# jasperlinthorst/reveal

Hardware: AMD Instinct MI355X
Metric: Mbp/s indexed+MUM-anchored (reveal rem) (higher is better)
Workload: dtype int32

## Files before the change

### reveal_amd/csrc/rv_cascade.hip

```cpp
#include "rv_index.h"
#include "rv_cascade.h"
#include "rv_leaf.h"
#include <algorithm>
#include <string.h>
#include <stdio.h>
#include <stdlib.h>
#include <chrono>

namespace {

constexpr int TB = 256;
constexpr u32 NONE = 0xFFFFFFFFu;
#ifdef RV_SA64
constexpr int KEY_SHIFT = 40;
#else
constexpr int KEY_SHIFT = 32;
#endif
constexpr u64 KEY_LOW = (1ull << KEY_SHIFT) - 1;

struct CasIv { sa_t a0, a1, b0, b1; };
struct CasRes { sa_t qa, qb; u32 ql, lead, trail, state; };
enum { C_NCHILD = 0, C_NUND = 1, C_NWIT = 2, C_ERR = 3, C_MAXN = 4, C_LO = 5, C_HI = 6, C_LEVELS = 7, C_NSOLVED = 8, C_NUNSOLVED = 9, C_NRETRY = 10, C_TICKET = 11,
       C_NANCH = 12  };

__device__ inline bool cas_cut(const CasIv &iv, int64_t pa, int64_t pb, int64_t len, int64_t minl, int64_t *qa, int64_t *qb, int64_t *ql) {
    const int64_t ka = (int64_t)iv.a0 - pa, kb = (int64_t)iv.b0 - pb;
    int64_t k = ka > kb ? ka : kb;
    k = k > 0 ? k : 0;
    const int64_t a = pa + k, b = pb + k;
    int64_t l = len - k;
    const int64_t ra = (int64_t)iv.a1 - a, rb = (int64_t)iv.b1 - b;
    l = l < ra ? l : ra;
    l = l < rb ? l : rb;
    *qa = a; *qb = b; *ql = l;
    return l >= minl;
}
__device__ inline u64 cas_key(int64_t qa, int64_t ql) { return ((u64)ql << KEY_SHIFT) | (KEY_LOW - (u64)qa); }

__device__ inline u64 shfl_up64(u64 v, int d) {
    const u32 lo = __shfl_up((u32)v, d, 64), hi = __shfl_up((u32)(v >> 32), d, 64);
    return ((u64)hi << 32) | lo;
}
__device__ inline void seg_atomic_max64(u64 *__restrict__ dst, u32 child, u64 val, bool active) {
    const int lane = threadIdx.x & 63;
    if (!active) { child = NONE; val = 0; }
    val = rv_wave_seg_max_u64(child, val);
    const u32 nc = __shfl_down(child, 1, 64);
    const bool last = lane == 63 || nc != child;
    if (active && last && val > dst[child]) atomicMax((unsigned long long *)&dst[child], (unsigned long long)val);
}
__device__ inline void seg_atomic_max32(u32 *__restrict__ dst, u32 child, u32 val, bool active) {
    const int lane = threadIdx.x & 63;
    if (!active) { child = NONE; val = 0; }
    val = rv_wave_seg_max_u32(child, val);
    const u32 nc = __shfl_down(child, 1, 64);
    const bool last = lane == 63 || nc != child;
    if (active && last && val > dst[child]) atomicMax(&dst[child], val);
}

constexpr int WT_ITEMS = 8;
constexpr int WT_TILE = TB * WT_ITEMS;
constexpr int WT_REGIONS = RV_WIT_REGIONS;
__global__ __launch_bounds__(TB) void k_cas_witness(const sa_t *__restrict__ SA, const lcp_t *__restrict__ LCP, const uint8_t *__restrict__ BWT, int64_t n,
                                                    u32 minl, sa_t *__restrict__ w_pos, u32 *__restrict__ w_val, u32 *__restrict__ w_rank, u32 cap , u32 *__restrict__ counters ) {
    __shared__ __attribute__((aligned(16))) u32 sl0[WT_TILE + 8];
    __shared__ __attribute__((aligned(16))) uint8_t ss0[WT_TILE + 32];
    u32 *const sl = sl0 + 3;
    uint8_t *const ss = ss0 + 15;
    const int64_t j0 = (int64_t)blockIdx.x * WT_TILE;
    if (j0 + WT_TILE + 2 <= n && sizeof(lcp_t) == 4) {
        const uint4 *L4 = reinterpret_cast<const uint4 *>(LCP + j0);
        uint4 *d4 = reinterpret_cast<uint4 *>(sl + 1);
        for (int k = threadIdx.x; k < WT_TILE / 4; k += TB) d4[k] = L4[k];
        const uint4 *B4 = reinterpret_cast<const uint4 *>(BWT + j0);
        for (int k = threadIdx.x; k < WT_TILE / 16; k += TB) {
            uint4 v = B4[k];
            v.x = (v.x >> 7) & 0x01010101u; v.y = (v.y >> 7) & 0x01010101u; v.z = (v.z >> 7) & 0x01010101u; v.w = (v.w >> 7) & 0x01010101u;
            reinterpret_cast<uint4 *>(ss + 1)[k] = v;
        }
        if (threadIdx.x == 0) { sl[0] = j0 > 0 ? (u32)LCP[j0 - 1] : 0u; ss[0] = j0 > 0 ? (uint8_t)(BWT[j0 - 1] >> 7) : (uint8_t)0; }
        if (threadIdx.x == 1) { sl[WT_TILE + 1] = (u32)LCP[j0 + WT_TILE]; ss[WT_TILE + 1] = (uint8_t)(BWT[j0 + WT_TILE] >> 7); }
        if (threadIdx.x == 2) sl[WT_TILE + 2] = (u32)LCP[j0 + WT_TILE + 1];
    } else {
        for (int k = threadIdx.x; k < WT_TILE + 3; k += TB) { const int64_t j = j0 - 1 + k; sl[k] = (j >= 0 && j < n) ? (u32)LCP[j] : 0u; }
        for (int k = threadIdx.x; k < WT_TILE + 2; k += TB) { const int64_t j = j0 - 1 + k; ss[k] = (j >= 0 && j < n) ? (uint8_t)(BWT[j] >> 7) : (uint8_t)0; }
    }
    __syncthreads();
    const int lane = threadIdx.x & 63;
    const u64 lt = (lane == 0) ? 0ull : (~0ull >> (64 - lane));
#pragma unroll 1
// ... 101 lines not shown
    if (i < NW) {
        const int64_t pos = (int64_t)w_pos[i];
        const bool a_side = t.nB == 0 || pos < (int64_t)t.beginB[0];
        const int ct = a_side ? cas_contig_of(t.beginA, t.nA, pos) : cas_contig_of(t.beginB, t.nB, pos);
        u32 c = NONE;
        if (ct >= 0) {
            const int32_t k = a_side ? t.pickA[ct] : t.pickB[ct];
            if (k >= 0) {
                for (int which = 0; which < 2 && c == NONE; which++) {
                    const u32 r = which ? t.rootTrail[k] : t.rootLead[k];
                    if (r == NONE) continue;
                    const CasIv p = roots[r];
                    if ((pos >= (int64_t)p.a0 && pos < (int64_t)p.a1) || (pos >= (int64_t)p.b0 && pos < (int64_t)p.b1)) c = r;
                }
            }
        }
        w_child[i] = c;
    }
}
__global__ void k_cas_lineage_stats(unsigned long long *__restrict__ stats, unsigned long long steps, unsigned long long maxdepth) {
    if (threadIdx.x == 0 && blockIdx.x == 0) { atomicAdd(&stats[0], steps); atomicMax(&stats[3], maxdepth); }
}
__global__ __launch_bounds__(TB) void k_cas_lkeys(const sa_t *__restrict__ c_pa, const u32 *__restrict__ c_len, u32 M, u64 *__restrict__ keys, u32 *__restrict__ vals) {
    const u32 i = blockIdx.x * TB + threadIdx.x;
    if (i < M) { keys[i] = (((1ull << (64 - KEY_SHIFT)) - 1ull - (u64)c_len[i]) << KEY_SHIFT) | (u64)c_pa[i]; vals[i] = i; }
}
__global__ __launch_bounds__(TB) void k_cas_lgather(const sa_t *__restrict__ c_pa, const sa_t *__restrict__ c_pb, const u32 *__restrict__ c_len, const u32 *__restrict__ perm, u32 M,
                                                    sa_t *__restrict__ o_pa, sa_t *__restrict__ o_pb, u32 *__restrict__ o_len) {
    const u32 i = blockIdx.x * TB + threadIdx.x;
    if (i < M) { const u32 f = perm[i]; o_pa[i] = c_pa[f]; o_pb[i] = c_pb[f]; o_len[i] = c_len[f]; }
}

constexpr int CAS_ITEMS = 4;
__global__ __launch_bounds__(TB) void k_cas_assign(const sa_t *__restrict__ c_pa, const sa_t *__restrict__ c_pb, const u32 *__restrict__ c_len, u32 *__restrict__ c_child,
                                                   u32 M, const sa_t *__restrict__ w_pos, const u32 *__restrict__ w_val, u32 *__restrict__ w_child, u32 NW,
                                                   const CasIv *__restrict__ iv, const CasRes *__restrict__ res, u64 *__restrict__ best, u32 *__restrict__ wmax,
                                                   int64_t minl, int first, const u64 *__restrict__ ceil ) {
    const u32 mblocks = (M + TB * CAS_ITEMS - 1) / (TB * CAS_ITEMS);
    for (int it = 0; it < CAS_ITEMS; it++) {
    if (blockIdx.x < mblocks) {
        const u32 i = (blockIdx.x * CAS_ITEMS + (u32)it) * TB + threadIdx.x;
        u32 c = i < M ? c_child[i] : NONE;
        bool live = c != NONE;
        u64 key = 0;
        if (live) {
            const int64_t pa = (int64_t)c_pa[i], pb = (int64_t)c_pb[i], len = (int64_t)c_len[i];
            int64_t qa, qb, ql;
            if (!first) {
                const CasRes r = res[c];
                const CasIv p = iv[c];
                u32 nc = NONE;
                if (r.state == 1u) {
                    CasIv lv; lv.a0 = p.a0; lv.a1 = r.qa; lv.b0 = p.b0; lv.b1 = r.qb;
                    CasIv tv; tv.a0 = (sa_t)((int64_t)r.qa + r.ql); tv.a1 = p.a1; tv.b0 = (sa_t)((int64_t)r.qb + r.ql); tv.b1 = p.b1;
                    if (r.lead != NONE && cas_cut(lv, pa, pb, len, minl, &qa, &qb, &ql)) nc = r.lead;
                    else if (r.trail != NONE && cas_cut(tv, pa, pb, len, minl, &qa, &qb, &ql)) nc = r.trail;
                } else if (r.state == 3u) {
                    if (cas_cut(p, pa, pb, len, minl, &qa, &qb, &ql)) nc = r.lead;
                }
                c = nc;
                c_child[i] = c;
                live = c != NONE;
            } else {
                live = cas_cut(iv[c], pa, pb, len, minl, &qa, &qb, &ql);
                if (!live) { c = NONE; c_child[i] = NONE; }
            }
            if (live) key = cas_key(qa, ql);
        }
        bool bid = live;
        if (live && ceil) { const u64 ce = ceil[c]; bid = ce == 0 || key < ce; }
        seg_atomic_max64(best, c, key, bid);
    } else {
        const u32 i = ((blockIdx.x - mblocks) * CAS_ITEMS + (u32)it) * TB + threadIdx.x;
        u32 c = i < NW ? w_child[i] : NONE;
        bool live = c != NONE;
        u32 v = 0;
        if (live) {
            const int64_t pos = (int64_t)w_pos[i];
            v = w_val[i];
            if (!first) {
                const CasRes r = res[c];
                const CasIv p = iv[c];
                u32 nc = NONE;
                if (r.state == 1u) {
                    const int64_t ea = (int64_t)r.qa + r.ql, eb = (int64_t)r.qb + r.ql;
                    const bool in_lead = (pos >= p.a0 && pos < r.qa) || (pos >= p.b0 && pos < r.qb);
                    const bool in_trail = (pos >= ea && pos < p.a1) || (pos >= eb && pos < p.b1);
                    nc = in_lead ? r.lead : in_trail ? r.trail : NONE;
                } else if (r.state == 3u) nc = r.lead;
                c = nc;
                w_child[i] = c;
                live = c != NONE;
            } else {
                const CasIv p = iv[c];
                live = (pos >= p.a0 && pos < p.a1) || (pos >= p.b0 && pos < p.b1);
                if (!live) { c = NONE; w_child[i] = NONE; }
            }
        }
        seg_atomic_max32(wmax, c, v, live);
    }
    }
}

__global__ __launch_bounds__(TB) void k_cas_winner(const sa_t *__restrict__ c_pa, const sa_t *__restrict__ c_pb, const u32 *__restrict__ c_len,
                                                   const u32 *__restrict__ c_child, u32 M, const CasIv *__restrict__ iv, CasRes *__restrict__ res,
                                                   const u64 *__restrict__ best, int64_t minl) {
    const u32 i = blockIdx.x * TB + threadIdx.x;
    if (i >= M) return;
    const u32 c = c_child[i];
    if (c == NONE) return;
    int64_t qa, qb, ql;
    if (!cas_cut(iv[c], (int64_t)c_pa[i], (int64_t)c_pb[i], (int64_t)c_len[i], minl, &qa, &qb, &ql)) return;
    if (cas_key(qa, ql) == best[c]) { res[c].qa = (sa_t)qa; res[c].qb = (sa_t)qb; res[c].ql = (u32)ql; }
}

constexpr u32 DWALK = 1024;
struct CasDanger { u64 *best; u32 *flag; sa_t *qb; u64 *ceil; u32 *m1, *p1, *m2; u64 *key; const uint8_t *T0; const lcp_t *LCP; const u64 *rank; u32 leaf_n; uint8_t *dflag; const uint8_t *wcls; };
__device__ inline bool cas_is_danger(const CasIv &p, u64 bk, u32 wm, u32 minl, u32 leaf_n, u32 *theta) {
    const int64_t la = (int64_t)p.a1 - p.a0, lb = (int64_t)p.b1 - p.b0;
    const u32 bl = (u32)(bk >> KEY_SHIFT);
    const bool can = (la >= (int64_t)minl) & (lb >= (int64_t)minl);
    const bool split = can & (bl >= minl) & (bl > wm);
    *theta = bl >= minl ? bl : minl;
    return can & !split & (wm >= minl) & ((u64)(la + lb) > (u64)leaf_n);
}
__global__ __launch_bounds__(TB) void k_cas_dmark(const CasIv *__restrict__ iv, const u64 *__restrict__ best, const u32 *__restrict__ wmax, u32 minl, const u32 *__restrict__ counters, CasDanger dg) {
    const u32 lo = counters[C_LO], hi = counters[C_HI];
    for (u32 id = lo + blockIdx.x * TB + threadIdx.x; id < hi; id += gridDim.x * TB) {
        u32 theta;
        dg.dflag[id] = cas_is_danger(iv[id], best[id], wmax[id], minl, dg.leaf_n, &theta) ? 1 : 0;
    }
}
__global__ __launch_bounds__(TB) void k_cas_dwalk(const sa_t *__restrict__ w_pos, const u32 *__restrict__ w_val, const u32 *__restrict__ w_child, u32 NW,
                                                  const CasIv *__restrict__ iv, const u64 *__restrict__ best, const u32 *__restrict__ wmax, u32 minl, CasDanger dg) {
    const u32 i = blockIdx.x * TB + threadIdx.x;
    if (i >= NW) return;
    if (dg.wcls && dg.wcls[i]) return;
    const u32 c = w_child[i];
    if (c == NONE || !dg.dflag[c]) return;
    dg.m1[i] = 0; dg.key[i] = 0;
    const CasIv p = iv[c];
    u32 theta;
    if (!cas_is_danger(p, best[c], wmax[c], minl, dg.leaf_n, &theta)) return;
    const int64_t pos = (int64_t)w_pos[i];
    const int64_t cap = (pos < (int64_t)p.a1 ? (int64_t)p.a1 : (int64_t)p.b1) - pos;
    if (w_val[i] < theta || cap < (int64_t)theta) return;
    u32 b1 = 0, b2 = 0, part = NONE;
    bool over = false;
#pragma unroll 1
    for (int dir = -1; dir <= 1; dir += 2) {
        u32 steps = 0;
        u64 rk = dg.rank[i];
        u32 run = 0xFFFFFFFFu;
        for (int64_t k = (int64_t)i + dir; k >= 0 && k < (int64_t)NW; k += dir) {
            const u64 r2 = dg.rank[k];
            if (r2 != rk + (u64)(int64_t)dir) break;
            const u32 g = (u32)dg.LCP[dir > 0 ? r2 : rk];
            run = g < run ? g : run;
            rk = r2;
            if (run < theta) break;
            if (++steps > DWALK) { over = true; break; }
            if (w_child[k] != c || w_val[k] < theta) continue;
            const int64_t pk = (int64_t)w_pos[k];
            const int64_t ck = (pk < (int64_t)p.a1 ? (int64_t)p.a1 : (int64_t)p.b1) - pk;
            if (ck < (int64_t)theta) continue;
            u32 l = (u32)(cap < ck ? cap : ck);
            l = run < l ? run : l;
            if (l > b1) { b2 = b1; b1 = l; part = (u32)k; }
            else if (l > b2) b2 = l;
// ... 3 lines not shown
    if (over) atomicOr(&dg.flag[c], 2u);
    dg.m1[i] = b1 >= theta ? b1 : 0u; dg.p1[i] = part; dg.m2[i] = b2;
}
constexpr u32 BLK_MIN = 64, BLK_MAX = 1024;
__global__ __launch_bounds__(TB) void k_cas_blk_flags(const u64 *__restrict__ rank, const lcp_t *__restrict__ LCP, u32 NW, u32 minl, u32 *__restrict__ flag) {
    const u32 i = blockIdx.x * TB + threadIdx.x;
    if (i >= NW) return;
    flag[i] = (i == 0 || rank[i] != rank[i - 1] + 1 || (u32)LCP[rank[i]] < minl) ? 1u : 0u;
}
__global__ __launch_bounds__(TB) void k_cas_blk_off(const u32 *__restrict__ flag, const u32 *__restrict__ bid, u32 NW, u32 nb, u32 *__restrict__ boff) {
    const u32 i = blockIdx.x * TB + threadIdx.x;
    if (i == 0) boff[nb] = NW;
    if (i < NW && flag[i]) boff[bid[i]] = i;
}
__global__ __launch_bounds__(TB) void k_cas_blk_class(const u32 *__restrict__ flag, const u32 *__restrict__ bid, const u32 *__restrict__ boff, u32 NW, u32 *__restrict__ mflag, uint8_t *__restrict__ wcls) {
    const u32 i = blockIdx.x * TB + threadIdx.x;
    if (i >= NW) return;
    const u32 b = bid[i] + flag[i] - 1u;
    const u32 size = boff[b + 1] - boff[b];
    const bool med = size > BLK_MIN && size <= BLK_MAX;
    wcls[i] = med ? 1 : 0;
    if (flag[i]) mflag[b] = med ? 1u : 0u;
}
__global__ __launch_bounds__(TB) void k_cas_blk_list(const u32 *__restrict__ mflag, const u32 *__restrict__ mid, u32 nb, u32 *__restrict__ mlist) {
    const u32 b = blockIdx.x * TB + threadIdx.x;
    if (b < nb && mflag[b]) mlist[mid[b]] = b;
}
__global__ __launch_bounds__(TB) void k_cas_dwalk_blk(const sa_t *__restrict__ w_pos, const u32 *__restrict__ w_val, const u32 *__restrict__ w_child, const u32 *__restrict__ boff,
                                                      const u32 *__restrict__ mlist, u32 nmed, const CasIv *__restrict__ iv, const u64 *__restrict__ best, const u32 *__restrict__ wmax,
                                                      u32 minl, CasDanger dg) {
    __shared__ u32 cc[BLK_MAX], vv[BLK_MAX], ll[BLK_MAX];
    __shared__ sa_t pp[BLK_MAX];
    __shared__ u32 s_any;
    const u32 b = mlist[blockIdx.x];
    const u32 s0 = boff[b], size = boff[b + 1] - s0;
    if (threadIdx.x == 0) s_any = 0;
    __syncthreads();
    bool any = false;
    for (u32 j = threadIdx.x; j < size; j += TB) {
        const u32 c = w_child[s0 + j];
        cc[j] = c;
        any |= c != NONE && dg.dflag[c];
    }
    if (__ballot(any) && (threadIdx.x & 63) == 0) s_any = 1;
    __syncthreads();
    if (!s_any) return;
    for (u32 j = threadIdx.x; j < size; j += TB) {
        vv[j] = w_val[s0 + j]; pp[j] = w_pos[s0 + j];
        ll[j] = (u32)dg.LCP[dg.rank[s0 + j]];
    }
    __syncthreads();
    for (u32 j = threadIdx.x; j < size; j += TB) {
        const u32 c = cc[j];
        if (c == NONE || !dg.dflag[c]) continue;
        const u32 i = s0 + j;
        dg.m1[i] = 0; dg.key[i] = 0;
        const CasIv p = iv[c];
        u32 theta;
        if (!cas_is_danger(p, best[c], wmax[c], minl, dg.leaf_n, &theta)) continue;
        const int64_t pos = (int64_t)pp[j];
        const int64_t cap = (pos < (int64_t)p.a1 ? (int64_t)p.a1 : (int64_t)p.b1) - pos;
        if (vv[j] < theta || cap < (int64_t)theta) continue;
        u32 b1 = 0, b2 = 0, part = NONE;
#pragma unroll 1
        for (int dir = -1; dir <= 1; dir += 2) {
            u32 run = 0xFFFFFFFFu;
            for (int64_t k = (int64_t)j + dir; k >= 0 && k < (int64_t)size; k += dir) {
                const u32 g = ll[dir > 0 ? k : k + 1];
                run = g < run ? g : run;
                if (run < theta) break;
                if (cc[k] != c || vv[k] < theta) continue;
                const int64_t pk = (int64_t)pp[k];
                const int64_t ck = (pk < (int64_t)p.a1 ? (int64_t)p.a1 : (int64_t)p.b1) - pk;
                if (ck < (int64_t)theta) continue;
                u32 l = (u32)(cap < ck ? cap : ck);
                l = run < l ? run : l;
                if (l > b1) { b2 = b1; b1 = l; part = s0 + (u32)k; }
                else if (l > b2) b2 = l;
                if (run <= b2) break;
            }
        }
        dg.m1[i] = b1 >= theta ? b1 : 0u; dg.p1[i] = part; dg.m2[i] = b2;
    }
}
__global__ __launch_bounds__(TB) void k_cas_dpick(const sa_t *__restrict__ w_pos, const u32 *__restrict__ w_val, const u32 *__restrict__ w_child, u32 NW,
                                                  const CasIv *__restrict__ iv, const CasRes *__restrict__ res, const u64 *__restrict__ best, const u32 *__restrict__ wmax,
                                                  u32 minl, CasDanger dg) {
    const u32 i = blockIdx.x * TB + threadIdx.x;
    if (i >= NW) return;
    const u32 c = w_child[i];
    if (c == NONE || !dg.dflag[c]) return;
    const CasIv p = iv[c];
    u32 theta;
    const u64 bk = best[c];
    if (!cas_is_danger(p, bk, wmax[c], minl, dg.leaf_n, &theta)) return;
    const int64_t pos = (int64_t)w_pos[i];
    const int64_t cap = (pos < (int64_t)p.a1 ? (int64_t)p.a1 : (int64_t)p.b1) - pos;
    if (w_val[i] < theta || cap < (int64_t)theta) return;
    if ((u32)(bk >> KEY_SHIFT) >= minl) { const CasRes r = res[c]; if (pos == (int64_t)r.qa || pos == (int64_t)r.qb) atomicOr(&dg.flag[c], 1u); }
    const u32 b1 = dg.m1[i];
    if (b1 == 0) return;
    const u32 w = dg.p1[i];
    if (dg.m1[w] != b1 || dg.p1[w] != i || b1 <= dg.m2[i] || b1 <= dg.m2[w]) return;
    const int64_t pw = (int64_t)w_pos[w];
    const bool a_side = pos < (int64_t)p.a1, w_a_side = pw < (int64_t)p.a1;
    if (!a_side || w_a_side) return;
    const int64_t qa = pos, qb = pw;
    if (!(qa == (int64_t)p.a0 || qb == (int64_t)p.b0)) {
        const uint8_t ca = dg.T0[qa - 1];
        if (ca == dg.T0[qb - 1] && ca != 'N' && ca != '$' && !(ca >= 'a' && ca <= 'z')) return;
    }
    const u64 key = cas_key(qa, (int64_t)b1);
    dg.key[i] = key;
    if (key > dg.best[c]) atomicMax((unsigned long long *)&dg.best[c], (unsigned long long)key);
}
__global__ __launch_bounds__(TB) void k_cas_dwrite(const sa_t *__restrict__ w_pos, const u32 *__restrict__ w_child, u32 NW, CasDanger dg) {
    const u32 i = blockIdx.x * TB + threadIdx.x;
    if (i >= NW) return;
    const u32 c = w_child[i];
    if (c == NONE || !dg.dflag[c]) return;
    const u64 key = dg.key[i];
    if (key == 0) return;
    if (key == dg.best[c]) dg.qb[c] = w_pos[dg.p1[i]];
}

__global__ __launch_bounds__(TB) void k_cas_decide(CasIv *__restrict__ iv, u64 *__restrict__ best, u32 *__restrict__ wmax, int32_t *__restrict__ depth,
                                                   CasRes *__restrict__ res, u32 minl, u32 *__restrict__ counters, u32 child_cap,
                                                   u32 *__restrict__ und_list, u32 leaf_n, RvCascadeIO io, CasDanger dg, int danger) {
    __shared__ u32 s_cnt[TB / 64][3];
    __shared__ u32 s_base[3];
    const u32 lo = counters[C_LO], hi = counters[C_HI];
    const int lane = threadIdx.x & 63, w = threadIdx.x >> 6;
    const u64 lt = (lane == 0) ? 0ull : (~0ull >> (64 - lane));
    for (u32 first = lo + blockIdx.x * TB; first < hi; first += gridDim.x * TB) {
        const u32 id = first + threadIdx.x;
        const bool in = id < hi;
        CasIv p; p.a0 = p.a1 = p.b0 = p.b1 = 0;
        u64 bk = 0; u32 wm = 0; int32_t dp = 0;
        CasRes r; r.qa = r.qb = 0; r.ql = 0; r.lead = r.trail = NONE; r.state = 2;
        if (in) { p = iv[id]; bk = best[id]; wm = wmax[id]; dp = depth[id]; r = res[id]; }
        const int64_t la = (int64_t)p.a1 - p.a0, lb = (int64_t)p.b1 - p.b0;
        const u32 bl = (u32)(bk >> KEY_SHIFT);
        const bool can = in & (la >= (int64_t)minl) & (lb >= (int64_t)minl);
        bool split = can & (bl >= minl) & (bl > wm);
        bool und = can & !split & (wm >= minl);
        bool forced = false, retry = false;
        if (danger && und && (u64)(la + lb) > (u64)dg.leaf_n) {
            const u32 fl = dg.flag[id];
            const u64 kh = dg.best[id], kc = (bl >= minl && !(fl & 1u)) ? bk : 0ull;
            if (!(fl & 2u)) {
                if (kh == 0 && kc == 0) {
                    if (bl < minl) und = false;
                    else if ((fl >> 8) < 16u) { retry = true; und = false; }
                } else {
                    if (kh > kc) { r.qa = (sa_t)(KEY_LOW - (kh & KEY_LOW)); r.qb = dg.qb[id]; r.ql = (u32)(kh >> KEY_SHIFT); }
                    split = true; forced = true; und = false;
                }
            }
// ... 512 lines not shown
            }
        }
        dg.leaf_n = (u32)ws.opt.cascade_danger_min;
    }
    const sa_t *d_beginA = nullptr, *d_beginB = nullptr;
    if (!chain) {
        hipLaunchKernelGGL(k_cas_init, dim3((unsigned)std::max<int64_t>(1, ceil_div((int64_t)NW, TB))), dim3(TB), 0, q, biv.as<CasIv>(), bbest.as<u64>(), bwm.as<u32>(),
                           bdep.as<int32_t>(), bres.as<CasRes>(), counters, root, bwc.as<u32>(), NW, dg.best, dg.flag, dg.ceil);
        RV_LAUNCH_CHECK();
    } else {
        const u32 R = cb.lin_roots, P = cb.lin_picks;
        if ((int64_t)R + 16 > (int64_t)ccap_k || P > iok.anchor_cap) GIVE_UP("more sequences than the cascade's tables hold");
        const uint8_t *tb = cb.d[32].as<uint8_t>();
        CasRootTabs rt;
        rt.beginA = (const sa_t *)(tb + cb.lin_off[0]); rt.beginB = (const sa_t *)(tb + cb.lin_off[1]);
        rt.pickA = (const int32_t *)(tb + cb.lin_off[2]); rt.pickB = (const int32_t *)(tb + cb.lin_off[3]);
        rt.rootLead = (const u32 *)(tb + cb.lin_off[4]); rt.rootTrail = (const u32 *)(tb + cb.lin_off[5]);
        rt.nA = cb.lin_nA; rt.nB = cb.lin_nB;
        d_beginA = rt.beginA; d_beginB = rt.beginB;
        hipLaunchKernelGGL(k_cas_init_roots, dim3((unsigned)std::max<int64_t>(1, ceil_div((int64_t)R, TB))), dim3(TB), 0, q, biv.as<CasIv>(), bbest.as<u64>(), bwm.as<u32>(),
                           bdep.as<int32_t>(), bres.as<CasRes>(), counters, (const CasIv *)cb.d[30].as<CasIv>(), (const int32_t *)cb.d[31].as<int32_t>(), R, dg.best, dg.flag, dg.ceil);
        RV_LAUNCH_CHECK();
        hipLaunchKernelGGL(k_cas_assign_roots, dim3((unsigned)std::max<int64_t>(1, ceil_div((int64_t)std::max(M, NW), TB))), dim3(TB), 0, q, (const sa_t *)bpa.as<sa_t>(),
                           (const sa_t *)bpb.as<sa_t>(), (const u32 *)blen.as<u32>(), bcc.as<u32>(), M, wp, bwc.as<u32>(), NW, (const CasIv *)cb.d[30].as<CasIv>(), rt, (int64_t)minl);
        RV_LAUNCH_CHECK();
        RV_HIP(hipMemcpyAsync(io.anchor_pos, cb.d[33].p, (size_t)P * 16, hipMemcpyDeviceToDevice, q));
        RV_HIP(hipMemcpyAsync(io.anchor_l, (const uint8_t *)cb.d[33].p + (size_t)P * 16, (size_t)P * 4, hipMemcpyDeviceToDevice, q));
        RV_HIP(hipMemcpyAsync(io.anchor_count, &cb.lin_picks, 4, hipMemcpyHostToDevice, q));
    }

    if (verbose) { (void)hipStreamSynchronize(q); tp[2] = cas_now(); }
    const unsigned agrid = (unsigned)(ceil_div((int64_t)M, TB * CAS_ITEMS) + ceil_div((int64_t)NW, TB * CAS_ITEMS));
    const int batch = std::max(1, (int)ws.opt.cascade_batch);
    int queued = 0;
    RV_TRY(rv_working_text_begin(h, host ? host->side : nullptr));
    u32 sent = 0, known = 0;
    auto send_known = [&]() -> int {
        if (!host || !host->side || !host->l || known <= sent || known > host->cap) return 0;
        RV_HIP(hipMemcpyAsync(host->pos + 2 * (size_t)sent, io.anchor_pos + 2 * (size_t)sent, (size_t)(known - sent) * 16, hipMemcpyDeviceToHost, host->side));
        RV_HIP(hipMemcpyAsync(host->l + sent, io.anchor_l + sent, (size_t)(known - sent) * 4, hipMemcpyDeviceToHost, host->side));
        sent = known;
        return 0;
    };
    struct PrioScope {
        Workspace &w; hipStream_t home; RvCascadeBufs &cb; bool on = false;
        ~PrioScope() { leave(); }
        void leave() {
            if (!on) return;
            on = false;
            (void)hipEventRecord(cb.ev_out, w.stream);
            w.stream = home;
            (void)hipStreamWaitEvent(home, cb.ev_out, 0);
        }
    } prio{ws, q, cb};
    if (ws.opt.cascade_prio) {
        if (!cb.prio_stream) {
            int plo = 0, phi = 0;
            RV_HIP(hipDeviceGetStreamPriorityRange(&plo, &phi));
            RV_HIP(hipStreamCreateWithPriority(&cb.prio_stream, hipStreamNonBlocking, phi));
            RV_HIP(hipEventCreateWithFlags(&cb.ev_in, hipEventDisableTiming));
            RV_HIP(hipEventCreateWithFlags(&cb.ev_out, hipEventDisableTiming));
        }
        RV_HIP(hipEventRecord(cb.ev_in, q));
        RV_HIP(hipStreamWaitEvent(cb.prio_stream, cb.ev_in, 0));
        ws.stream = cb.prio_stream; prio.on = true;
        q = cb.prio_stream;
    }
    for (;;) {
        for (int b = 0; b < batch; b++, queued++) {
            hipLaunchKernelGGL(k_cas_assign, dim3(agrid), dim3(TB), 0, q, (const sa_t *)bpa.as<sa_t>(), (const sa_t *)bpb.as<sa_t>(), (const u32 *)blen.as<u32>(), bcc.as<u32>(), M,
                               wp, wv, bwc.as<u32>(), NW, (const CasIv *)biv.as<CasIv>(), (const CasRes *)bres.as<CasRes>(),
                               bbest.as<u64>(), bwm.as<u32>(), (int64_t)minl, queued == 0 ? 1 : 0, (const u64 *)((danger && NW) ? dg.ceil : nullptr));
            RV_LAUNCH_CHECK();
            hipLaunchKernelGGL(k_cas_winner, dim3((unsigned)ceil_div((int64_t)M, TB)), dim3(TB), 0, q, (const sa_t *)bpa.as<sa_t>(), (const sa_t *)bpb.as<sa_t>(),
                               (const u32 *)blen.as<u32>(), (const u32 *)bcc.as<u32>(), M, (const CasIv *)biv.as<CasIv>(), bres.as<CasRes>(), (const u64 *)bbest.as<u64>(), (int64_t)minl);
            RV_LAUNCH_CHECK();
            if (danger && NW) {
                const unsigned wb = (unsigned)ceil_div((int64_t)NW, TB);
                hipLaunchKernelGGL(k_cas_dmark, dim3(256), dim3(TB), 0, q, (const CasIv *)biv.as<CasIv>(), (const u64 *)bbest.as<u64>(), (const u32 *)bwm.as<u32>(), minl, (const u32 *)counters, dg);
                RV_LAUNCH_CHECK();
                hipLaunchKernelGGL(k_cas_dwalk, dim3(wb), dim3(TB), 0, q, wp, wv, (const u32 *)bwc.as<u32>(), NW, (const CasIv *)biv.as<CasIv>(), (const u64 *)bbest.as<u64>(),
                                   (const u32 *)bwm.as<u32>(), minl, dg);
                RV_LAUNCH_CHECK();
                if (dwalk_nmed) {
                    hipLaunchKernelGGL(k_cas_dwalk_blk, dim3((unsigned)dwalk_nmed), dim3(TB), 0, q, wp, wv, (const u32 *)bwc.as<u32>(), dwalk_boff, dwalk_mlist, dwalk_nmed,
                                       (const CasIv *)biv.as<CasIv>(), (const u64 *)bbest.as<u64>(), (const u32 *)bwm.as<u32>(), minl, dg);
                    RV_LAUNCH_CHECK();
                }
                hipLaunchKernelGGL(k_cas_dpick, dim3(wb), dim3(TB), 0, q, wp, wv, (const u32 *)bwc.as<u32>(), NW, (const CasIv *)biv.as<CasIv>(), (const CasRes *)bres.as<CasRes>(),
                                   (const u64 *)bbest.as<u64>(), (const u32 *)bwm.as<u32>(), minl, dg);
                RV_LAUNCH_CHECK();
                hipLaunchKernelGGL(k_cas_dwrite, dim3(wb), dim3(TB), 0, q, wp, (const u32 *)bwc.as<u32>(), NW, dg);
                RV_LAUNCH_CHECK();
            }
            hipLaunchKernelGGL(k_cas_decide, dim3(256), dim3(TB), 0, q, biv.as<CasIv>(), bbest.as<u64>(), bwm.as<u32>(), bdep.as<int32_t>(),
                               bres.as<CasRes>(), minl, counters, ccap_k, bund.as<u32>(), (u32)RV_LEAF_N, iok, dg, (danger && NW) ? 1 : 0);
            RV_LAUNCH_CHECK();
        }
        RV_TRY(send_known());
        RV_TRY(rv_read_back(ws, hc, counters, sizeof hc));
        if (hc[C_ERR] & ~5u) { rv_set_error("cascade: device error %u", hc[C_ERR]); return -1; }
        if (hc[C_ERR]) GIVE_UP("the cascade's tables are full");
        known = hc[C_NANCH];
        if (hc[C_MAXN] > (u32)RV_LEAF_N) break;
        if (hc[C_HI] == hc[C_LO]) break;
        if (queued > 1000000) { rv_set_error("cascade: no progress"); return -1; }
    }
    prio.leave(); q = ws.stream;
    const int level = (int)hc[C_LEVELS];
    const u32 hi = hc[C_NCHILD];
    if (verbose) tp[3] = cas_now();
    out->levels = level; out->children = hi; out->solved = hc[C_NSOLVED]; out->unsolved = hc[C_NUNSOLVED];
    const u32 U = hc[C_NUND];
    out->undecided = U;
    if (hc[C_MAXN] > (u32)RV_LEAF_N) {
        out->why = "an undecided sub-index above the leaf kernel's size";
        if (verbose) fprintf(stderr, "cascade%s: gave up: %s (%u ranks; %u levels, %u sub-indices, %u undecided, %u decided from witnesses, %u not)\n", danger ? " (second attempt)" : "", out->why, hc[C_MAXN], level, hi, U, hc[C_NSOLVED], hc[C_NUNSOLVED]);
        return 0;
    }
    hipLaunchKernelGGL(k_cas_stats, dim3(256), dim3(TB), 0, q, (const u32 *)counters, (const int32_t *)bdep.as<int32_t>(), io);
    RV_LAUNCH_CHECK();
    RV_TRY(send_known());
    if (chain) {
        hipLaunchKernelGGL(k_cas_lineage_stats, dim3(1), dim3(64), 0, q, io.stats, (unsigned long long)cb.lin_steps, (unsigned long long)cb.lin_maxdepth);
        RV_LAUNCH_CHECK();
    }
    if (U > 0) {
        RV_TRY(bsz.reserve((size_t)(U + 1) * 8));
// ... 43 lines not shown
```

### reveal_amd/csrc/rv_common.h

```cpp
#pragma once
#include <algorithm>
#include <mutex>
#include <thread>
#include <vector>
#include <utility>
#include <hip/hip_runtime.h>
#include <stdint.h>
#include <string.h>
#include <stddef.h>
#include <vector>
#include <string>

#ifdef RV_SA64
typedef int64_t  sa_t;
typedef uint32_t lcp_t;
#else
typedef int32_t  sa_t;
typedef int32_t  lcp_t;
#endif

typedef unsigned long long u64;
typedef unsigned int       u32;

void rv_set_error(const char *fmt, ...);
// ... 9 lines not shown
#define RV_TRY(x)                                                                              \
    do {                                                                                       \
        int r_ = (x);                                                                          \
        if (r_ != 0) return r_;                                                                \
    } while (0)
#define RV_OPTION_LIST(X) \
    X(bubble_par_min, "RV_BUBBLE_PAR_MIN", -1) \
    X(presel_log, "RV_PRESEL_LOG", 0) \
    X(presel_host, "RV_PRESEL_HOST", 0) \
    X(leaf_acap, "RV_LEAF_ACAP", 256) \
    X(bubble_lds_always, "RV_BUBBLE_LDS_ALWAYS", 0) \
    X(no_early_bubble, "RV_NO_EARLY_BUBBLE", 0) \
    X(early_bubble_many, "RV_EARLY_BUBBLE_MANY", 0) \
    X(no_early_split, "RV_NO_EARLY_SPLIT", 0) \
    X(keep_dead, "RV_KEEP_DEAD", 0) \
    X(bubble_no_lds, "RV_BUBBLE_NO_LDS", 0) \
    X(bubble_no_join, "RV_BUBBLE_NO_JOIN", 0) \
    X(bubble_no_merge, "RV_BUBBLE_NO_MERGE", 0) \
    X(tables_memcpy, "RV_TABLES_MEMCPY", 0) \
    X(bubble_parent_scratch, "RV_BUBBLE_PARENT_SCRATCH", 0) \
    X(level_log, "RV_LEVEL_LOG", 0) \
    X(pb_two_pass, "RV_PB_TWO_PASS", 0) \
    X(no_leaf, "RV_NO_LEAF", 0) \
    X(leaf_prof, "RV_LEAF_PROF", 0) \
    X(no_cascade, "RV_NO_CASCADE", 0) \
    X(cascade_second, "RV_CASCADE_SECOND", 0) \
    X(cascade_danger, "RV_CASCADE_DANGER", 1) \
    X(cascade_second_off, "RV_CASCADE_SECOND_OFF", 0) \
    X(sync_block, "RV_SYNC_BLOCK", 0) \
    X(pb_refresh_tmin, "RV_PB_REFRESH_TMIN", 0) \
    X(cascade_log, "RV_CASCADE_LOG", 0) \
    X(cascade_danger_min, "RV_CASCADE_DANGER_MIN", 0) \
    X(cascade_batch, "RV_CASCADE_BATCH", 8) \
    X(lcp_by_rank, "RV_LCP_BY_RANK", 0) \
    X(no_tiny_sa, "RV_NO_TINY_SA", 0) \
    X(no_short_alphabet, "RV_NO_SHORT_ALPHABET", 0) \
    X(no_fused_lcp, "RV_NO_FUSED_LCP", 0) \
    X(no_diag, "RV_NO_DIAG", 0) \
    X(no_packed_text, "RV_NO_PACKED_TEXT", 0) \
    X(no_heads_fusion, "RV_NO_HEADS_FUSION", 0) \
    X(no_twin_collapse, "RV_NO_TWIN_COLLAPSE", 0) \
    X(no_far_twins, "RV_NO_FAR_TWINS", 0) \
    X(no_lcp_list, "RV_NO_LCP_LIST", 0) \
    X(no_text_jump, "RV_NO_TEXT_JUMP", 0) \
    X(far_table, "RV_FAR_TABLE", 0) \
    X(no_slow_class, "RV_NO_SLOW_CLASS", 0) \
    X(no_dwalk_blocks, "RV_NO_DWALK_BLOCKS", 0) \
    X(no_pub_twins, "RV_NO_PUB_TWINS", 0) \
    X(sa_no_text, "RV_SA_NO_TEXT", 0) \
    X(text_mode, "RV_TEXT_MODE", -1) \
    X(carry_ch, "RV_CARRY_CH", -1) \
    X(rs_bits, "RV_RS_BITS", 8) \
    X(rs_xcd, "RV_RS_XCD", 1) \
    X(rs_cnt16, "RV_RS_CNT16", 1) \
    X(rs_no_digit_bytes, "RV_RS_NO_DIGIT_BYTES", 0) \
    X(diag_table, "RV_DIAG_TABLE", -1) \
    X(no_cascade_chain, "RV_NO_CASCADE_CHAIN", 0) \
    X(casm_rank_count, "RV_CASM_RANK_COUNT", 0) \
    X(casm_big_min, "RV_CASM_BIG_MIN", -1) \
    X(casm_no_big, "RV_CASM_NO_BIG", 0) \
    X(casm_big_root, "RV_CASM_BIG_ROOT", 1 << 22) \
    X(casm_big_total, "RV_CASM_BIG_TOTAL", 1 << 26) \
    X(lock_any, "RV_LOCK_ANY", 0) \
    X(presel_dev_min, "RV_PRESEL_DEV_MIN", 65536) \
    X(scan_v1, "RV_SCAN_V1", 0) \
    X(pick_threads, "RV_PICK_THREADS", 0) \
// ... 328 lines not shown
```

Before: 23760.

## Skip empty cascade levels on device and aggregate uniform-wave best updates per block

Kernels in the batched cascade loop now read the level counters and exit early when a level is empty (lo==hi). The batched launches past convergence therefore become nearly free instead of re-running assign/winner/danger work. k_cas_assign is restructured: it prefetches child ids for all items, splits the segmented max from the atomic raise, and reads the current best before raising. Waves whose lanes all bid for one child defer their update to a block-level shared-memory reduction, which cuts global atomics on hot children. Decide grid size becomes a tunable knob with the same default. The extra counter read and __syncthreads add small overhead per launch.

Result: faster. 24240 (median of 6 runs) (+2.0%).

```diff
diff --git a/reveal_amd/csrc/rv_cascade.hip b/reveal_amd/csrc/rv_cascade.hip
--- a/reveal_amd/csrc/rv_cascade.hip
+++ b/reveal_amd/csrc/rv_cascade.hip
@@ -41,21 +41,27 @@
     const u32 lo = __shfl_up((u32)v, d, 64), hi = __shfl_up((u32)(v >> 32), d, 64);
     return ((u64)hi << 32) | lo;
 }
-__device__ inline void seg_atomic_max64(u64 *__restrict__ dst, u32 child, u64 val, bool active) {
+__device__ inline u64 seg_run_max64(u32 child, u64 val, bool active, bool *last) {
     const int lane = threadIdx.x & 63;
     if (!active) { child = NONE; val = 0; }
     val = rv_wave_seg_max_u64(child, val);
     const u32 nc = __shfl_down(child, 1, 64);
-    const bool last = lane == 63 || nc != child;
-    if (active && last && val > dst[child]) atomicMax((unsigned long long *)&dst[child], (unsigned long long)val);
-}
-__device__ inline void seg_atomic_max32(u32 *__restrict__ dst, u32 child, u32 val, bool active) {
+    *last = active && (lane == 63 || nc != child);
+    return val;
+}
+__device__ inline u32 seg_run_max32(u32 child, u32 val, bool active, bool *last) {
     const int lane = threadIdx.x & 63;
     if (!active) { child = NONE; val = 0; }
     val = rv_wave_seg_max_u32(child, val);
     const u32 nc = __shfl_down(child, 1, 64);
-    const bool last = lane == 63 || nc != child;
-    if (active && last && val > dst[child]) atomicMax(&dst[child], val);
+    *last = active && (lane == 63 || nc != child);
+    return val;
+}
+__device__ inline void seg_raise64(u64 *dst, u32 child, u64 val, u64 seen, bool last) {
+    if (last && val > seen) atomicMax((unsigned long long *)&dst[child], (unsigned long long)val);
+}
+__device__ inline void seg_raise32(u32 *dst, u32 child, u32 val, u32 seen, bool last) {
+    if (last && val > seen) atomicMax(&dst[child], val);
 }
 
 constexpr int WT_ITEMS = 8;
@@ -223,90 +229,168 @@
 }
 
 constexpr int CAS_ITEMS = 4;
+constexpr int CAS_GROUP = 1;
 __global__ __launch_bounds__(TB) void k_cas_assign(const sa_t *__restrict__ c_pa, const sa_t *__restrict__ c_pb, const u32 *__restrict__ c_len, u32 *__restrict__ c_child,
                                                    u32 M, const sa_t *__restrict__ w_pos, const u32 *__restrict__ w_val, u32 *__restrict__ w_child, u32 NW,
                                                    const CasIv *__restrict__ iv, const CasRes *__restrict__ res, u64 *__restrict__ best, u32 *__restrict__ wmax,
-                                                   int64_t minl, int first, const u64 *__restrict__ ceil ) {
+                                                   int64_t minl, int first, const u64 *__restrict__ ceil ,
+                                                   const u32 *__restrict__ counters) {
+    __shared__ u64 s_val[CAS_ITEMS][TB / 64];
+    __shared__ u32 s_ch[CAS_ITEMS][TB / 64];
     const u32 mblocks = (M + TB * CAS_ITEMS - 1) / (TB * CAS_ITEMS);
-    for (int it = 0; it < CAS_ITEMS; it++) {
-    if (blockIdx.x < mblocks) {
-        const u32 i = (blockIdx.x * CAS_ITEMS + (u32)it) * TB + threadIdx.x;
-        u32 c = i < M ? c_child[i] : NONE;
-        bool live = c != NONE;
-        u64 key = 0;
-        if (live) {
-            const int64_t pa = (int64_t)c_pa[i], pb = (int64_t)c_pb[i], len = (int64_t)c_len[i];
-            int64_t qa, qb, ql;
-            if (!first) {
-                const CasRes r = res[c];
-                const CasIv p = iv[c];
-                u32 nc = NONE;
-                if (r.state == 1u) {
-                    CasIv lv; lv.a0 = p.a0; lv.a1 = r.qa; lv.b0 = p.b0; lv.b1 = r.qb;
-                    CasIv tv; tv.a0 = (sa_t)((int64_t)r.qa + r.ql); tv.a1 = p.a1; tv.b0 = (sa_t)((int64_t)r.qb + r.ql); tv.b1 = p.b1;
-                    if (r.lead != NONE && cas_cut(lv, pa, pb, len, minl, &qa, &qb, &ql)) nc = r.lead;
-                    else if (r.trail != NONE && cas_cut(tv, pa, pb, len, minl, &qa, &qb, &ql)) nc = r.trail;
-                } else if (r.state == 3u) {
-                    if (cas_cut(p, pa, pb, len, minl, &qa, &qb, &ql)) nc = r.lead;
+    const bool mhalf = blockIdx.x < mblocks;
+    const u32 i0 = (mhalf ? blockIdx.x : blockIdx.x - mblocks) * (u32)(CAS_ITEMS * TB) + threadIdx.x;
+    const u32 cnt = mhalf ? M : NW;
+    u32 *const child = mhalf ? c_child : w_child;
+    u32 c[CAS_ITEMS];
+#pragma unroll
+    for (int it = 0; it < CAS_ITEMS; it++) { const u32 i = i0 + (u32)it * TB; c[it] = i < cnt ? child[i] : NONE; }
+    if (!first && counters[C_LO] == counters[C_HI]) return;
+#pragma unroll
+    for (int g = 0; g < CAS_ITEMS; g += CAS_GROUP) {
+        const u32 ig = i0 + (u32)g * TB;
+        u32 *const cg = c + g;
+        CasRes r[CAS_GROUP];
+        CasIv p[CAS_GROUP];
+        if (mhalf) {
+            sa_t pa[CAS_GROUP], pb[CAS_GROUP];
+            u32 len[CAS_GROUP];
+#pragma unroll
+            for (int it = 0; it < CAS_GROUP; it++) {
+                pa[it] = 0; pb[it] = 0; len[it] = 0;
+                p[it].a0 = p[it].a1 = p[it].b0 = p[it].b1 = 0;
+                r[it].qa = r[it].qb = 0; r[it].ql = 0; r[it].lead = r[it].trail = NONE; r[it].state = 2;
+                if (cg[it] != NONE) {
+                    const u32 i = ig + (u32)it * TB;
+                    pa[it] = c_pa[i]; pb[it] = c_pb[i]; len[it] = c_len[i];
+                    p[it] = iv[cg[it]];
+                    if (!first) r[it] = res[cg[it]];
                 }
-                c = nc;
-                c_child[i] = c;
-                live = c != NONE;
-            } else {
-                live = cas_cut(iv[c], pa, pb, len, minl, &qa, &qb, &ql);
-                if (!live) { c = NONE; c_child[i] = NONE; }
-            }
-            if (live) key = cas_key(qa, ql);
-        }
-        bool bid = live;
-        if (live && ceil) { const u64 ce = ceil[c]; bid = ce == 0 || key < ce; }
-        seg_atomic_max64(best, c, key, bid);
-    } else {
-        const u32 i = ((blockIdx.x - mblocks) * CAS_ITEMS + (u32)it) * TB + threadIdx.x;
-        u32 c = i < NW ? w_child[i] : NONE;
-        bool live = c != NONE;
-        u32 v = 0;
-        if (live) {
-            const int64_t pos = (int64_t)w_pos[i];
-            v = w_val[i];
-            if (!first) {
-                const CasRes r = res[c];
-                const CasIv p = iv[c];
-                u32 nc = NONE;
-                if (r.state == 1u) {
-                    const int64_t ea = (int64_t)r.qa + r.ql, eb = (int64_t)r.qb + r.ql;
-                    const bool in_lead = (pos >= p.a0 && pos < r.qa) || (pos >= p.b0 && pos < r.qb);
-                    const bool in_trail = (pos >= ea && pos < p.a1) || (pos >= eb && pos < p.b1);
-                    nc = in_lead ? r.lead : in_trail ? r.trail : NONE;
-                } else if (r.state == 3u) nc = r.lead;
-                c = nc;
-                w_child[i] = c;
-                live = c != NONE;
-            } else {
-                const CasIv p = iv[c];
-                live = (pos >= p.a0 && pos < p.a1) || (pos >= p.b0 && pos < p.b1);
-                if (!live) { c = NONE; w_child[i] = NONE; }
-            }
-        }
-        seg_atomic_max32(wmax, c, v, live);
-    }
+            }
+            u64 key[CAS_GROUP], ce[CAS_GROUP];
+            bool live[CAS_GROUP];
+#pragma unroll
+            for (int it = 0; it < CAS_GROUP; it++) {
+                const u32 i = ig + (u32)it * TB;
+                live[it] = cg[it] != NONE;
+                key[it] = 0; ce[it] = 0;
+                if (live[it]) {
+                    const int64_t a = (int64_t)pa[it], b = (int64_t)pb[it], l = (int64_t)len[it];
+                    int64_t qa, qb, ql;
+                    if (!first) {
+                        u32 nc = NONE;
+                        if (r[it].state == 1u) {
+                            CasIv lv; lv.a0 = p[it].a0; lv.a1 = r[it].qa; lv.b0 = p[it].b0; lv.b1 = r[it].qb;
+                            CasIv tv; tv.a0 = (sa_t)((int64_t)r[it].qa + r[it].ql); tv.a1 = p[it].a1; tv.b0 = (sa_t)((int64_t)r[it].qb + r[it].ql); tv.b1 = p[it].b1;
+                            if (r[it].lead != NONE && cas_cut(lv, a, b, l, minl, &qa, &qb, &ql)) nc = r[it].lead;
+                            else if (r[it].trail != NONE && cas_cut(tv, a, b, l, minl, &qa, &qb, &ql)) nc = r[it].trail;
+                        } else if (r[it].state == 3u) {
+                            if (cas_cut(p[it], a, b, l, minl, &qa, &qb, &ql)) nc = r[it].lead;
+                        }
+                        cg[it] = nc;
+                        c_child[i] = nc;
+                        live[it] = nc != NONE;
+                    } else {
+                        live[it] = cas_cut(p[it], a, b, l, minl, &qa, &qb, &ql);
+                        if (!live[it]) { cg[it] = NONE; c_child[i] = NONE; }
+                    }
+                    if (live[it]) {
+                        key[it] = cas_key(qa, ql);
+                        if (ceil) ce[it] = ceil[cg[it]];
+                    }
+                }
+            }
+            u64 seen[CAS_GROUP];
+            bool last[CAS_GROUP];
+#pragma unroll
+            for (int it = 0; it < CAS_GROUP; it++) {
+                const bool bid = live[it] && (ce[it] == 0 || key[it] < ce[it]);
+                key[it] = seg_run_max64(cg[it], key[it], bid, &last[it]);
+                const bool whole = __all(bid && cg[it] == (u32)__shfl((int)cg[it], 0, 64));
+                if ((threadIdx.x & 63) == 63) { s_ch[g + it][threadIdx.x >> 6] = whole ? cg[it] : NONE; s_val[g + it][threadIdx.x >> 6] = key[it]; }
+                if (whole) last[it] = false;
+                seen[it] = last[it] ? best[cg[it]] : 0;
+            }
+#pragma unroll
+            for (int it = 0; it < CAS_GROUP; it++) seg_raise64(best, cg[it], key[it], seen[it], last[it]);
+        } else {
+            sa_t pos[CAS_GROUP];
+            u32 v[CAS_GROUP];
+#pragma unroll
+            for (int it = 0; it < CAS_GROUP; it++) {
+                pos[it] = 0; v[it] = 0;
+                p[it].a0 = p[it].a1 = p[it].b0 = p[it].b1 = 0;
+                r[it].qa = r[it].qb = 0; r[it].ql = 0; r[it].lead = r[it].trail = NONE; r[it].state = 2;
+                if (cg[it] != NONE) {
+                    const u32 i = ig + (u32)it * TB;
+                    pos[it] = w_pos[i]; v[it] = w_val[i];
+                    p[it] = iv[cg[it]];
+                    if (!first) r[it] = res[cg[it]];
+                }
+            }
+            u32 seen[CAS_GROUP];
+            bool last[CAS_GROUP];
+#pragma unroll
+            for (int it = 0; it < CAS_GROUP; it++) {
+                const u32 i = ig + (u32)it * TB;
+                bool live = cg[it] != NONE;
+                if (live) {
+                    const int64_t ps = (int64_t)pos[it];
+                    if (!first) {
+                        u32 nc = NONE;
+                        if (r[it].state == 1u) {
+                            const int64_t ea = (int64_t)r[it].qa + r[it].ql, eb = (int64_t)r[it].qb + r[it].ql;
+                            const bool in_lead = (ps >= p[it].a0 && ps < r[it].qa) || (ps >= p[it].b0 && ps < r[it].qb);
+                            const bool in_trail = (ps >= ea && ps < p[it].a1) || (ps >= eb && ps < p[it].b1);
+                            nc = in_lead ? r[it].lead : in_trail ? r[it].trail : NONE;
+                        } else if (r[it].state == 3u) nc = r[it].lead;
+                        cg[it] = nc;
+                        w_child[i] = nc;
+                        live = nc != NONE;
+                    } else {
+                        live = (ps >= p[it].a0 && ps < p[it].a1) || (ps >= p[it].b0 && ps < p[it].b1);
+                        if (!live) { cg[it] = NONE; w_child[i] = NONE; }
+                    }
+                }
+                v[it] = seg_run_max32(cg[it], v[it], live, &last[it]);
+                seen[it] = last[it] ? wmax[cg[it]] : 0;
+            }
+#pragma unroll
+            for (int it = 0; it < CAS_GROUP; it++) seg_raise32(wmax, cg[it], v[it], seen[it], last[it]);
+        }
+    }
+    if (mhalf) {
+        __syncthreads();
+        if (threadIdx.x < 64) {
+            const u32 l = threadIdx.x;
+            const u32 ch = l < (u32)(CAS_ITEMS * (TB / 64)) ? s_ch[l / (TB / 64)][l % (TB / 64)] : NONE;
+            u64 v = ch != NONE ? s_val[l / (TB / 64)][l % (TB / 64)] : 0;
+            bool last;
+            v = seg_run_max64(ch, v, ch != NONE, &last);
+            seg_raise64(best, ch, v, last ? best[ch] : 0, last);
+        }
     }
 }
 
 __global__ __launch_bounds__(TB) void k_cas_winner(const sa_t *__restrict__ c_pa, const sa_t *__restrict__ c_pb, const u32 *__restrict__ c_len,
                                                    const u32 *__restrict__ c_child, u32 M, const CasIv *__restrict__ iv, CasRes *__restrict__ res,
-                                                   const u64 *__restrict__ best, int64_t minl) {
-    const u32 i = blockIdx.x * TB + threadIdx.x;
-    if (i >= M) return;
-    const u32 c = c_child[i];
+                                                   const u64 *__restrict__ best, int64_t minl, const u32 *__restrict__ counters) {
+    const u32 i = blockIdx.x * TB + threadIdx.x;
+    const u32 c = i < M ? c_child[i] : NONE;
+    if (counters[C_LO] == counters[C_HI]) return;
     if (c == NONE) return;
+    const CasIv p = iv[c];
+    const u64 bk = best[c];
+    const int64_t pa = (int64_t)c_pa[i], pb = (int64_t)c_pb[i], len = (int64_t)c_len[i];
     int64_t qa, qb, ql;
-    if (!cas_cut(iv[c], (int64_t)c_pa[i], (int64_t)c_pb[i], (int64_t)c_len[i], minl, &qa, &qb, &ql)) return;
-    if (cas_key(qa, ql) == best[c]) { res[c].qa = (sa_t)qa; res[c].qb = (sa_t)qb; res[c].ql = (u32)ql; }
+    if (!cas_cut(p, pa, pb, len, minl, &qa, &qb, &ql)) return;
+    if (cas_key(qa, ql) == bk) { res[c].qa = (sa_t)qa; res[c].qb = (sa_t)qb; res[c].ql = (u32)ql; }
 }
 
 constexpr u32 DWALK = 1024;
-struct CasDanger { u64 *best; u32 *flag; sa_t *qb; u64 *ceil; u32 *m1, *p1, *m2; u64 *key; const uint8_t *T0; const lcp_t *LCP; const u64 *rank; u32 leaf_n; uint8_t *dflag; const uint8_t *wcls; };
+struct CasDanger { u64 *best; u32 *flag; sa_t *qb; u64 *ceil; u32 *m1, *p1, *m2; u64 *key; const uint8_t *T0; const lcp_t *LCP; const u64 *rank; u32 leaf_n; uint8_t *dflag; const uint8_t *wcls;
+                   const u32 *ctr;  };
+__device__ inline bool cas_level_empty(const CasDanger &dg) { return dg.ctr[C_LO] == dg.ctr[C_HI]; }
 __device__ inline bool cas_is_danger(const CasIv &p, u64 bk, u32 wm, u32 minl, u32 leaf_n, u32 *theta) {
     const int64_t la = (int64_t)p.a1 - p.a0, lb = (int64_t)p.b1 - p.b0;
     const u32 bl = (u32)(bk >> KEY_SHIFT);
@@ -325,7 +409,7 @@
 __global__ __launch_bounds__(TB) void k_cas_dwalk(const sa_t *__restrict__ w_pos, const u32 *__restrict__ w_val, const u32 *__restrict__ w_child, u32 NW,
                                                   const CasIv *__restrict__ iv, const u64 *__restrict__ best, const u32 *__restrict__ wmax, u32 minl, CasDanger dg) {
     const u32 i = blockIdx.x * TB + threadIdx.x;
-    if (i >= NW) return;
+    if (i >= NW || cas_level_empty(dg)) return;
     if (dg.wcls && dg.wcls[i]) return;
     const u32 c = w_child[i];
     if (c == NONE || !dg.dflag[c]) return;
@@ -395,6 +479,7 @@
     __shared__ u32 cc[BLK_MAX], vv[BLK_MAX], ll[BLK_MAX];
     __shared__ sa_t pp[BLK_MAX];
     __shared__ u32 s_any;
+    if (cas_level_empty(dg)) return;
     const u32 b = mlist[blockIdx.x];
     const u32 s0 = boff[b], size = boff[b + 1] - s0;
     if (threadIdx.x == 0) s_any = 0;
@@ -450,7 +535,7 @@
                                                   const CasIv *__restrict__ iv, const CasRes *__restrict__ res, const u64 *__restrict__ best, const u32 *__restrict__ wmax,
                                                   u32 minl, CasDanger dg) {
     const u32 i = blockIdx.x * TB + threadIdx.x;
-    if (i >= NW) return;
+    if (i >= NW || cas_level_empty(dg)) return;
     const u32 c = w_child[i];
     if (c == NONE || !dg.dflag[c]) return;
     const CasIv p = iv[c];
@@ -479,7 +564,7 @@
 }
 __global__ __launch_bounds__(TB) void k_cas_dwrite(const sa_t *__restrict__ w_pos, const u32 *__restrict__ w_child, u32 NW, CasDanger dg) {
     const u32 i = blockIdx.x * TB + threadIdx.x;
-    if (i >= NW) return;
+    if (i >= NW || cas_level_empty(dg)) return;
     const u32 c = w_child[i];
     if (c == NONE || !dg.dflag[c]) return;
     const u64 key = dg.key[i];
@@ -487,6 +572,7 @@
     if (key == dg.best[c]) dg.qb[c] = w_pos[dg.p1[i]];
 }
 
+constexpr unsigned DEC_GRID = 256;
 __global__ __launch_bounds__(TB) void k_cas_decide(CasIv *__restrict__ iv, u64 *__restrict__ best, u32 *__restrict__ wmax, int32_t *__restrict__ depth,
                                                    CasRes *__restrict__ res, u32 minl, u32 *__restrict__ counters, u32 child_cap,
                                                    u32 *__restrict__ und_list, u32 leaf_n, RvCascadeIO io, CasDanger dg, int danger) {
@@ -1065,6 +1151,8 @@
     if (verbose) { (void)hipStreamSynchronize(q); tp[2] = cas_now(); }
     const unsigned agrid = (unsigned)(ceil_div((int64_t)M, TB * CAS_ITEMS) + ceil_div((int64_t)NW, TB * CAS_ITEMS));
     const int batch = std::max(1, (int)ws.opt.cascade_batch);
+    const unsigned dgrid = ws.opt.cas_decide_grid > 0 ? (unsigned)std::min<int64_t>(ws.opt.cas_decide_grid, 65536) : DEC_GRID;
+    dg.ctr = counters;
     int queued = 0;
     RV_TRY(rv_working_text_begin(h, host ? host->side : nullptr));
     u32 sent = 0, known = 0;
@@ -1103,10 +1191,10 @@
         for (int b = 0; b < batch; b++, queued++) {
             hipLaunchKernelGGL(k_cas_assign, dim3(agrid), dim3(TB), 0, q, (const sa_t *)bpa.as<sa_t>(), (const sa_t *)bpb.as<sa_t>(), (const u32 *)blen.as<u32>(), bcc.as<u32>(), M,
                                wp, wv, bwc.as<u32>(), NW, (const CasIv *)biv.as<CasIv>(), (const CasRes *)bres.as<CasRes>(),
-                               bbest.as<u64>(), bwm.as<u32>(), (int64_t)minl, queued == 0 ? 1 : 0, (const u64 *)((danger && NW) ? dg.ceil : nullptr));
+                               bbest.as<u64>(), bwm.as<u32>(), (int64_t)minl, queued == 0 ? 1 : 0, (const u64 *)((danger && NW) ? dg.ceil : nullptr), (const u32 *)counters);
             RV_LAUNCH_CHECK();
             hipLaunchKernelGGL(k_cas_winner, dim3((unsigned)ceil_div((int64_t)M, TB)), dim3(TB), 0, q, (const sa_t *)bpa.as<sa_t>(), (const sa_t *)bpb.as<sa_t>(),
-                               (const u32 *)blen.as<u32>(), (const u32 *)bcc.as<u32>(), M, (const CasIv *)biv.as<CasIv>(), bres.as<CasRes>(), (const u64 *)bbest.as<u64>(), (int64_t)minl);
+                               (const u32 *)blen.as<u32>(), (const u32 *)bcc.as<u32>(), M, (const CasIv *)biv.as<CasIv>(), bres.as<CasRes>(), (const u64 *)bbest.as<u64>(), (int64_t)minl, (const u32 *)counters);
             RV_LAUNCH_CHECK();
             if (danger && NW) {
                 const unsigned wb = (unsigned)ceil_div((int64_t)NW, TB);
@@ -1126,7 +1214,7 @@
                 hipLaunchKernelGGL(k_cas_dwrite, dim3(wb), dim3(TB), 0, q, wp, (const u32 *)bwc.as<u32>(), NW, dg);
                 RV_LAUNCH_CHECK();
             }
-            hipLaunchKernelGGL(k_cas_decide, dim3(256), dim3(TB), 0, q, biv.as<CasIv>(), bbest.as<u64>(), bwm.as<u32>(), bdep.as<int32_t>(),
+            hipLaunchKernelGGL(k_cas_decide, dim3(dgrid), dim3(TB), 0, q, biv.as<CasIv>(), bbest.as<u64>(), bwm.as<u32>(), bdep.as<int32_t>(),
                                bres.as<CasRes>(), minl, counters, ccap_k, bund.as<u32>(), (u32)RV_LEAF_N, iok, dg, (danger && NW) ? 1 : 0);
             RV_LAUNCH_CHECK();
         }
diff --git a/reveal_amd/csrc/rv_common.h b/reveal_amd/csrc/rv_common.h
--- a/reveal_amd/csrc/rv_common.h
+++ b/reveal_amd/csrc/rv_common.h
@@ -65,6 +65,7 @@
     X(cascade_log, "RV_CASCADE_LOG", 0) \
     X(cascade_danger_min, "RV_CASCADE_DANGER_MIN", 0) \
     X(cascade_batch, "RV_CASCADE_BATCH", 8) \
+    X(cas_decide_grid, "RV_CAS_DECIDE_GRID", 0) \
     X(lcp_by_rank, "RV_LCP_BY_RANK", 0) \
     X(no_tiny_sa, "RV_NO_TINY_SA", 0) \
     X(no_short_alphabet, "RV_NO_SHORT_ALPHABET", 0) \
```
